# markomih/SplatFields

Measured on AMD Instinct MI355X. Metric: splats*px rasterized/sec (fwd+bwd), higher is better.
Workload: dtype f32

## Files before the change

include/splatraster.h:

```cpp
#ifndef SPLATRASTER_H
#define SPLATRASTER_H

#include <stddef.h>

#ifdef __cplusplus
extern "C" {
#endif

#define SR_VERSION 4
#define SR_TILE 16

typedef struct SrView {
    int image_height;
    int image_width;
    float tanfovx;
    float tanfovy;
    float scale_modifier;
    int sh_degree;
    int sh_coeffs;
    int prefiltered;
    int debug;
    const float* viewmatrix;
    const float* projmatrix;
    const float* campos;
// ... 21 lines not shown
typedef struct SrGrads {
    float* dL_dmeans3D;
    float* dL_dmeans2D;
    float* dL_dopacity;
    float* dL_dscales;
    float* dL_drotations;
    float* dL_dcov3D;
    float* dL_dshs;
    float* dL_dcolors;
    float* dL_dshs_rest;
} SrGrads;

int sr_version(void);
const char* sr_last_error(void);

size_t sr_geom_bytes(int n_splats, int height, int width);
size_t sr_binning_bytes(long long instances, int height, int width);
size_t sr_image_bytes(int height, int width);
size_t sr_backward_scratch_bytes(long long instances);

int sr_forward_prepare(const SrView* view, const SrSplats* splats, void* geom, int* radii,
                       long long* instances_out, void* hip_stream);

int sr_forward_render(const SrView* view, const SrSplats* splats, void* geom, void* binning,
                      long long instances, void* image, float* out_color, float* out_depth,
                      float* out_alpha, void* hip_stream);

#define SR_NEED_CAPACITY 2
int sr_forward(const SrView* view, const SrSplats* splats, void* geom, int* radii, void* binning,
               long long binning_capacity, void* image, float* out_color, float* out_depth, float* out_alpha,
               long long* instances_out, void* hip_stream);

int sr_forward_async(const SrView* view, const SrSplats* splats, void* geom, int* radii, void* binning,
                     long long binning_capacity, long long longest_list_hint, long long longest_list_expected, void* image,
                     float* out_color, float* out_depth, float* out_alpha, void** ticket_out, void* hip_stream);
int sr_ticket_wait(void* ticket, long long* instances_out, long long* longest_list_out);
long long sr_last_longest_list(void);
int sr_ticket_release(void* ticket);

#define SR_BWD_SLOT_SPEC_BELOW 6
int sr_backward(const SrView* view, const SrSplats* splats, const void* geom, void* binning,
                long long instances, long long instances_rendered, const void* image, const int* radii,
                const float* dL_dcolor, const float* dL_ddepth, const float* dL_dalpha, void* scratch,
                const SrGrads* grads, void* hip_stream);

int sr_backward_blend(const SrView* view, const SrSplats* splats, const void* geom, void* binning,
                      long long instances, long long instances_rendered, const void* image,
                      const float* dL_dcolor, const float* dL_ddepth, const float* dL_dalpha, void* scratch, void* hip_stream);
int sr_backward_splats(const SrView* view, const SrSplats* splats, const void* geom, void* binning,
                       long long instances, long long instances_rendered, const void* image, const int* radii, void* scratch,
                       const SrGrads* grads, int first_splat, int n_splats, void* hip_stream);

int sr_set_backward_kernel(int which);

int sr_mark_visible(int n_splats, const float* means3D, const float* viewmatrix,
                    const float* projmatrix, unsigned char* present, void* hip_stream);

int sr_densification_stats(int n_splats, const float* dL_dmeans2D, const int* radii, float* grad_accum, float* denom,
                           float* max_radii2D, void* hip_stream);

size_t sr_loss_workspace_bytes(int planes, int height, int width);
size_t sr_loss_maps_bytes(int planes, int height, int width);
int sr_photometric_forward(int batch, int channels, int height, int width, const float* image, const float* gt,
                           const float* alpha, const float* gt_mask, float lambda_dssim, float lambda_mask, void* workspace,
                           float* maps, float* loss, float* l1, float* ssim, float* mask_l1, void* hip_stream);
int sr_photometric_backward(int batch, int channels, int height, int width, const float* image, const float* gt,
                            const float* alpha, const float* gt_mask, const float* maps, float w_l1, float w_ssim, float w_mask,
                            const float* upstream, int upstream_per_item, float* dL_dimage, float* dL_dalpha, void* hip_stream);

#define SR_QUANT_NONE 0
#define SR_QUANT_PNG 1
#define SR_QUANT_TO8B 2
size_t sr_metrics_workspace_bytes(int batch, int height, int width);
int sr_image_metrics(int batch, int height, int width, const float* pred, const long long* pred_strides4, const float* gt,
                     const long long* gt_strides4, const float* mask, long long mask_item_stride, int quantize, void* workspace,
                     float* psnr, float* ssim, float* psnr_channels, unsigned char* frames, void* hip_stream);

int sr_sh_forward(int n_splats, int sh_coeffs, int sh_degree, const float* means3D, const float* shs, const float* campos,
                  float* colors, unsigned char* clamped, void* hip_stream);

int sr_sh_forward_views(int n_splats, int sh_coeffs, int sh_degree, int n_views, const float* means3D, const float* shs,
                        const float* campos, float* colors, float* keep, void* hip_stream);

int sr_sh_backward(int n_splats, int sh_coeffs, int sh_degree, int n_views, const float* means3D, const float* shs,
                   const float* campos, const float* dL_dcolors, float scale, float* dL_dshs, float* dL_dmeans3D,
                   int accumulate_means, void* hip_stream);

size_t sr_knn_workspace_bytes(int n_points);
int sr_knn3_mean_dist2(int n_points, const float* points, float* mean_dist2, void* workspace, void* hip_stream);

#define SR_KNN_MAX_K 8
size_t sr_knn_graph_workspace_bytes(int n_points, int k);
int sr_knn_graph(int n_points, int k, const float* points, int* nn_ix, unsigned* order, unsigned* rev_start, unsigned* rev_edges,
                 void* workspace, void* hip_stream);

#define SR_MORAN_MAX_TENSORS 8
size_t sr_moran_workspace_bytes(int n_items, int n_tensors);
size_t sr_moran_edges_bytes(int n_items, int k, int channels);
int sr_moran_forward(int n_items, int k, float eps, const float* points, const float* weight, const int* nn_ix,
                     const unsigned* order, int n_tensors, const float* const* features, const int* widths, void* workspace,
                     float* out, void* hip_stream);
int sr_moran_backward(int n_items, int k, float eps, const float* points, const float* weight, const int* nn_ix,
                      const unsigned* order, const unsigned* rev_start, const unsigned* rev_edges, int n_tensors,
                      const float* const* features, const int* widths, const float* out, const float* upstream, void* edges,
                      float* const* dL_dfeatures, float* dL_dpoints, float* dL_dweight, void* hip_stream);
int sr_moran_weights(int n_points, int k, float eps, const float* points, const int* nn_ix, float* weights, void* hip_stream);
// ... 200 lines not shown
```

splatfields_amd/_lib.py:

```python
from __future__ import annotations

import ctypes as C
from pathlib import Path

import os

import torch

LIB_PATH = Path(os.environ.get("SPLATRASTER_LIB") or (Path(__file__).resolve().parent / "libsplatraster.so"))

c_float_p = C.c_void_p


class SrView(C.Structure):
    _fields_ = [("image_height", C.c_int), ("image_width", C.c_int), ("tanfovx", C.c_float), ("tanfovy", C.c_float),
                ("scale_modifier", C.c_float), ("sh_degree", C.c_int), ("sh_coeffs", C.c_int), ("prefiltered", C.c_int),
                ("debug", C.c_int), ("viewmatrix", C.c_void_p), ("projmatrix", C.c_void_p), ("campos", C.c_void_p),
                ("bg", C.c_void_p)]


class SrSplats(C.Structure):
    _fields_ = [("count", C.c_int), ("means3D", C.c_void_p), ("opacities", C.c_void_p), ("scales", C.c_void_p),
                ("rotations", C.c_void_p), ("cov3D_precomp", C.c_void_p), ("shs", C.c_void_p),
                ("colors_precomp", C.c_void_p), ("raw_params", C.c_int), ("shs_rest", C.c_void_p)]
# ... 38 lines not shown

class SrPlaneJob(C.Structure):
    _fields_ = [(name, C.c_void_p) for name in (
        "x", "weight", "bias", "gamma", "beta", "stats", "residual", "out", "pre", "dy", "dx", "dweight", "dbias", "dgamma", "dbeta",
        "d_residual", "add", "dx_out")]


class SrHullView(C.Structure):
    _fields_ = [("m", C.c_double * 12), ("mask_offset", C.c_longlong), ("height", C.c_int), ("width", C.c_int),
                ("convention", C.c_int), ("outside", C.c_int)]


HULL_KRT, HULL_NDC, HULL_OUTSIDE_CARVE, HULL_OUTSIDE_KEEP, HULL_MAX_VIEWS = 0, 1, 0, 1, 1024
RESFIELD_MAX_JOBS, RESFIELD_MAX_RANK = 16, 64
PLANE_MAX_JOBS = 8
CONV_PROLOGUE, CONV_UPSAMPLE, CONV_RESIDUAL, CONV_SILU_OUT = 1, 2, 4, 8
MLP_MAX_GRAD_JOBS, MLP_MAX_GRAD_TASKS = 16, 128
MLP_MAX_PACK_JOBS = 32
MORAN_MAX_TENSORS, KNN_MAX_K = 8, 8
ADAM_MAX_TENSORS = 32
QUANT_NONE, QUANT_PNG, QUANT_TO8B = 0, 1, 2
MLP_MAX_OPS, MLP_NONE, MLP_LEAKY, MLP_MASK = 24, 0, 1, 2


SYMBOLS = {
    "sr_version": (C.c_int, []),
    "sr_last_error": (C.c_char_p, []),
    "sr_geom_bytes": (C.c_size_t, [C.c_int, C.c_int, C.c_int]),
    "sr_binning_bytes": (C.c_size_t, [C.c_longlong, C.c_int, C.c_int]),
    "sr_image_bytes": (C.c_size_t, [C.c_int, C.c_int]),
    "sr_backward_scratch_bytes": (C.c_size_t, [C.c_longlong]),
    "sr_forward_prepare": (C.c_int, [C.POINTER(SrView), C.POINTER(SrSplats), C.c_void_p, C.c_void_p,
                                     C.POINTER(C.c_longlong), C.c_void_p]),
    "sr_forward_render": (C.c_int, [C.POINTER(SrView), C.POINTER(SrSplats), C.c_void_p, C.c_void_p, C.c_longlong,
                                    C.c_void_p, C.c_void_p, C.c_void_p, C.c_void_p, C.c_void_p]),
    "sr_forward": (C.c_int, [C.POINTER(SrView), C.POINTER(SrSplats), C.c_void_p, C.c_void_p, C.c_void_p, C.c_longlong,
                             C.c_void_p, C.c_void_p, C.c_void_p, C.c_void_p, C.POINTER(C.c_longlong), C.c_void_p]),
    "sr_forward_async": (C.c_int, [C.POINTER(SrView), C.POINTER(SrSplats), C.c_void_p, C.c_void_p, C.c_void_p, C.c_longlong,
                                   C.c_longlong, C.c_longlong, C.c_void_p, C.c_void_p, C.c_void_p, C.c_void_p, C.POINTER(C.c_void_p),
                                   C.c_void_p]),
    "sr_ticket_wait": (C.c_int, [C.c_void_p, C.POINTER(C.c_longlong), C.POINTER(C.c_longlong)]),
    "sr_ticket_release": (C.c_int, [C.c_void_p]),
    "sr_last_longest_list": (C.c_longlong, []),
    "sr_debug_counters": (C.c_int, [C.POINTER(C.c_longlong), C.c_int]),
    "sr_backward": (C.c_int, [C.POINTER(SrView), C.POINTER(SrSplats), C.c_void_p, C.c_void_p, C.c_longlong, C.c_longlong, C.c_void_p,
                              C.c_void_p, C.c_void_p, C.c_void_p, C.c_void_p, C.c_void_p, C.POINTER(SrGrads),
                              C.c_void_p]),
    "sr_backward_blend": (C.c_int, [C.POINTER(SrView), C.POINTER(SrSplats), C.c_void_p, C.c_void_p, C.c_longlong, C.c_longlong, C.c_void_p,
                                    C.c_void_p, C.c_void_p, C.c_void_p, C.c_void_p, C.c_void_p]),
    "sr_backward_splats": (C.c_int, [C.POINTER(SrView), C.POINTER(SrSplats), C.c_void_p, C.c_void_p, C.c_longlong, C.c_longlong, C.c_void_p, C.c_void_p,
                                     C.c_void_p, C.POINTER(SrGrads), C.c_int, C.c_int, C.c_void_p]),
    "sr_debug_snapshot": (C.c_int, [C.POINTER(SrView), C.POINTER(SrSplats), C.c_void_p, C.c_void_p, C.c_void_p, C.c_int]),
    "sr_set_backward_kernel": (C.c_int, [C.c_int]),
    "sr_sh_forward": (C.c_int, [C.c_int, C.c_int, C.c_int, C.c_void_p, C.c_void_p, C.c_void_p, C.c_void_p, C.c_void_p, C.c_void_p]),
    "sr_sh_forward_views": (C.c_int, [C.c_int, C.c_int, C.c_int, C.c_int, C.c_void_p, C.c_void_p, C.c_void_p, C.c_void_p, C.c_void_p, C.c_void_p]),
    "sr_sh_backward": (C.c_int, [C.c_int, C.c_int, C.c_int, C.c_int, C.c_void_p, C.c_void_p, C.c_void_p, C.c_void_p, C.c_float,
                                 C.c_void_p, C.c_void_p, C.c_int, C.c_void_p]),
    "sr_knn_workspace_bytes": (C.c_size_t, [C.c_int]),
    "sr_knn3_mean_dist2": (C.c_int, [C.c_int, C.c_void_p, C.c_void_p, C.c_void_p, C.c_void_p]),
    "sr_knn_graph_workspace_bytes": (C.c_size_t, [C.c_int, C.c_int]),
    "sr_knn_graph": (C.c_int, [C.c_int, C.c_int, C.c_void_p, C.c_void_p, C.c_void_p, C.c_void_p, C.c_void_p, C.c_void_p, C.c_void_p]),
    "sr_moran_workspace_bytes": (C.c_size_t, [C.c_int, C.c_int]),
    "sr_moran_edges_bytes": (C.c_size_t, [C.c_int, C.c_int, C.c_int]),
    "sr_moran_forward": (C.c_int, [C.c_int, C.c_int, C.c_float, C.c_void_p, C.c_void_p, C.c_void_p, C.c_void_p, C.c_int,
                                   C.POINTER(C.c_void_p), C.POINTER(C.c_int), C.c_void_p, C.c_void_p, C.c_void_p]),
    "sr_moran_backward": (C.c_int, [C.c_int, C.c_int, C.c_float, C.c_void_p, C.c_void_p, C.c_void_p, C.c_void_p, C.c_void_p, C.c_void_p,
                                    C.c_int, C.POINTER(C.c_void_p), C.POINTER(C.c_int), C.c_void_p, C.c_void_p, C.c_void_p,
                                    C.POINTER(C.c_void_p), C.c_void_p, C.c_void_p, C.c_void_p]),
    "sr_moran_weights": (C.c_int, [C.c_int, C.c_int, C.c_float, C.c_void_p, C.c_void_p, C.c_void_p, C.c_void_p]),
    "sr_moran_weights_backward": (C.c_int, [C.c_int, C.c_int, C.c_float, C.c_void_p, C.c_void_p, C.c_void_p, C.c_void_p, C.c_void_p,
                                            C.c_void_p, C.c_void_p, C.c_void_p]),
    "sr_loss_workspace_bytes": (C.c_size_t, [C.c_int, C.c_int, C.c_int]),
    "sr_loss_maps_bytes": (C.c_size_t, [C.c_int, C.c_int, C.c_int]),
    "sr_photometric_forward": (C.c_int, [C.c_int, C.c_int, C.c_int, C.c_int, C.c_void_p, C.c_void_p, C.c_void_p, C.c_void_p, C.c_float,
                                         C.c_float, C.c_void_p, C.c_void_p, C.c_void_p, C.c_void_p, C.c_void_p, C.c_void_p, C.c_void_p]),
    "sr_photometric_backward": (C.c_int, [C.c_int, C.c_int, C.c_int, C.c_int, C.c_void_p, C.c_void_p, C.c_void_p, C.c_void_p, C.c_void_p,
                                          C.c_float, C.c_float, C.c_float, C.c_void_p, C.c_int, C.c_void_p, C.c_void_p, C.c_void_p]),
    "sr_metrics_workspace_bytes": (C.c_size_t, [C.c_int, C.c_int, C.c_int]),
    "sr_image_metrics": (C.c_int, [C.c_int, C.c_int, C.c_int, C.c_void_p, C.POINTER(C.c_longlong), C.c_void_p, C.POINTER(C.c_longlong),
                                   C.c_void_p, C.c_longlong, C.c_int, C.c_void_p, C.c_void_p, C.c_void_p, C.c_void_p, C.c_void_p,
                                   C.c_void_p]),
    "sr_adam_step": (C.c_int, [C.c_int, C.POINTER(SrAdamJob), C.c_void_p, C.c_longlong, C.c_void_p]),
    "sr_splat_reg_workspace_bytes": (C.c_size_t, [C.c_int]),
    "sr_splat_reg_forward": (C.c_int, [C.c_int, C.c_void_p, C.c_void_p, C.c_double, C.c_double, C.c_double, C.c_void_p, C.c_void_p, C.c_void_p]),
    "sr_splat_reg_backward": (C.c_int, [C.c_int, C.c_void_p, C.c_void_p, C.c_double, C.c_double, C.c_double, C.c_void_p, C.c_void_p, C.c_void_p,
                                        C.c_void_p, C.c_void_p]),
    "sr_depth_l1_workspace_bytes": (C.c_size_t, [C.c_int, C.c_int, C.c_int]),
    "sr_depth_l1_forward": (C.c_int, [C.c_int, C.c_int, C.c_int, C.c_void_p, C.c_void_p, C.c_void_p, C.c_void_p, C.c_void_p]),
    "sr_depth_l1_backward": (C.c_int, [C.c_int, C.c_int, C.c_int, C.c_void_p, C.c_void_p, C.c_void_p, C.c_int, C.c_void_p, C.c_void_p]),
    "sr_densify_workspace_bytes": (C.c_size_t, [C.c_int]),
    "sr_densify_plan": (C.c_int, [C.c_int, C.c_void_p, C.c_int, C.c_void_p, C.c_void_p, C.c_void_p, C.c_void_p, C.c_float, C.c_float,
                                  C.c_float, C.c_float, C.c_float, C.c_void_p, C.c_void_p, C.POINTER(C.c_longlong), C.c_void_p]),
    "sr_densify_gather": (C.c_int, [C.c_int, C.c_int, C.c_void_p, C.c_void_p, C.c_void_p, C.c_int, C.c_void_p, C.c_int, C.c_void_p,
                                    C.c_void_p, C.c_void_p]),
    "sr_hull_workspace_bytes": (C.c_size_t, [C.c_longlong]),
    "sr_hull_carve": (C.c_int, [C.c_int, C.POINTER(SrHullView), C.c_void_p, C.c_longlong, C.c_void_p, C.c_int, C.c_void_p, C.c_longlong,
                                C.c_int, C.c_void_p, C.c_void_p, C.c_void_p]),
    "sr_hull_gather": (C.c_int, [C.c_void_p, C.c_int, C.c_void_p, C.c_longlong, C.c_int, C.c_void_p, C.c_longlong, C.c_void_p, C.c_void_p,
                                 C.c_void_p]),
    "sr_mlp_pack": (C.c_int, [C.c_int, C.POINTER(SrMlpPackJob), C.c_void_p]),
    "sr_mlp_weight_grad_workspace": (C.c_size_t, [C.c_int, C.c_int, C.POINTER(SrMlpGradJob)]),
    "sr_mlp_weight_grad": (C.c_int, [C.c_int, C.c_int, C.POINTER(SrMlpGradJob), C.c_void_p, C.c_size_t, C.c_void_p]),
    "sr_mlp_chain": (C.c_int, [C.c_int, C.c_int, C.c_int, C.POINTER(SrMlpOp), C.c_float, C.c_void_p]),
    "sr_mlp_pack_bf16": (C.c_int, [C.c_int, C.POINTER(SrMlpPackJob), C.c_void_p]),
    "sr_mlp_chain_bf16": (C.c_int, [C.c_int, C.c_int, C.c_int, C.POINTER(SrMlpOp), C.c_float, C.c_void_p]),
    "sr_mlp_input_forward": (C.c_int, [C.c_int, C.c_int, C.c_int, C.c_int, C.c_int, C.c_void_p, C.c_void_p, C.c_void_p, C.c_void_p, C.c_void_p]),
# ... 95 lines not shown
```

splatfields_amd/csrc/api.hip:

```cpp
#include <cstdint>
#include <cstdio>
#include <cstdlib>
#include <cstring>
#include <atomic>
#include <chrono>
#include <thread>
#include <mutex>
#include <string>
#include <vector>
#include "kernels.h"

namespace {

thread_local std::string g_last_error;
thread_local long long g_last_longest = -1;

int fail(const std::string& msg) { g_last_error = msg; return 1; }

int check_hip(hipError_t e, const char* what) {
    if (e == hipSuccess) return 0;
    return fail(std::string(what) + ": " + hipGetErrorString(e));
}

template <typename... P>
// ... 405 lines not shown
    const sr::SplatsK& s = c.s;
    float* slots = static_cast<float*>(scratch);
    if (what & 1) {
        StageTimer t_(5, st);
        const int pinned = g_bwd_kernel.load(std::memory_order_relaxed);
        const bool wave_kernel = pinned == 1;
        if (wave_kernel) sr::launch_render_backward(c.v, c.g, c.b, c.im, dL_dcolor, dL_ddepth, dL_dalpha, slots, st);
        else sr::launch_render_backward_quads(c.v, c.g, c.b, c.im, dL_dcolor, dL_ddepth, dL_dalpha, slots, st);
    }
    if (what & 1) SR_TRY(after_launch(view, st, "render_backward"));
    if (what & 2) {
        sr::GradsK gr;
        gr.means3D = grads->dL_dmeans3D; gr.means2D = grads->dL_dmeans2D; gr.opacity = grads->dL_dopacity;
        gr.scales = s.cov3D ? nullptr : grads->dL_dscales; gr.rotations = s.cov3D ? nullptr : grads->dL_drotations;
        gr.cov3D = s.cov3D ? grads->dL_dcov3D : nullptr;
        gr.shs = s.shs ? grads->dL_dshs : nullptr;
        gr.shs_rest = (s.shs_rest && gr.shs) ? grads->dL_dshs_rest : nullptr;
        gr.colors = (s.colors || (s.shs && !grads->dL_dshs)) ? grads->dL_dcolors : nullptr;
        const bool small_fp = !(instances_rendered >= 0 && instances_rendered > (long long)SR_BWD_SLOT_SPEC_BELOW * (long long)s.N);
        { StageTimer t_(6, st); sr::launch_preprocess_backward(c.v, s, c.g, radii, slots, c.b.reached, gr, first, count, small_fp, st); }
        SR_TRY(after_launch(view, st, "preprocess_backward"));
    }
    return 0;
}
}

int sr_backward(const SrView* view, const SrSplats* splats, const void* geom, void* binning,
                long long instances, long long instances_rendered, const void* image, const int* radii,
                const float* dL_dcolor, const float* dL_ddepth, const float* dL_dalpha, void* scratch,
                const SrGrads* grads, void* hip_stream) {
    return backward_impl(3, view, splats, geom, binning, instances, instances_rendered, image, radii, dL_dcolor, dL_ddepth, dL_dalpha,
                         scratch, grads, 0, splats ? splats->count : 0, hip_stream);
}

int sr_backward_blend(const SrView* view, const SrSplats* splats, const void* geom, void* binning,
                      long long instances, long long instances_rendered, const void* image,
                      const float* dL_dcolor, const float* dL_ddepth, const float* dL_dalpha, void* scratch, void* hip_stream) {
    return backward_impl(1, view, splats, geom, binning, instances, instances_rendered, image, nullptr, dL_dcolor, dL_ddepth, dL_dalpha,
                         scratch, nullptr, 0, 0, hip_stream);
}

int sr_backward_splats(const SrView* view, const SrSplats* splats, const void* geom, void* binning,
                       long long instances, long long instances_rendered, const void* image, const int* radii, void* scratch,
                       const SrGrads* grads, int first_splat, int n_splats, void* hip_stream) {
    return backward_impl(2, view, splats, geom, binning, instances, instances_rendered, image, radii, nullptr, nullptr, nullptr, scratch,
                         grads, first_splat, n_splats, hip_stream);
}

int sr_set_backward_kernel(int which) {
    if (which < 0 || which > 2) return -1;
    return g_bwd_kernel.exchange(which, std::memory_order_relaxed);
}

int sr_mark_visible(int n, const float* means3D, const float* viewmatrix, const float*, unsigned char* present, void* hip_stream) {
    if (n < 0 || (n > 0 && (!means3D || !viewmatrix || !present))) return fail("bad arguments to sr_mark_visible");
    hipStream_t st = static_cast<hipStream_t>(hip_stream);
    sr::launch_mark_visible(n, means3D, viewmatrix, present, st);
    return check_hip(hipGetLastError(), "mark_visible");
}

int sr_densification_stats(int n, const float* dL_dmeans2D, const int* radii, float* grad_accum, float* denom, float* max_radii2D,
                           void* hip_stream) {
    if (n < 0) return fail("bad arguments to sr_densification_stats");
    if (n > 0 && (!dL_dmeans2D || !radii)) return fail("null pointer in sr_densification_stats");
    sr::launch_densification_stats(n, dL_dmeans2D, radii, grad_accum, denom, max_radii2D, static_cast<hipStream_t>(hip_stream));
    return check_hip(hipGetLastError(), "densification_stats");
}

int sr_sh_forward(int n, int sh_coeffs, int sh_degree, const float* means3D, const float* shs, const float* campos,
                  float* colors, unsigned char* clamped, void* hip_stream) {
    if (n < 0 || sh_degree < 0 || sh_degree > 3 || sh_coeffs < (sh_degree + 1) * (sh_degree + 1)) return fail("bad arguments to sr_sh_forward");
    if (n > 0 && (!means3D || !shs || !campos || !colors || !clamped)) return fail("null pointer in sr_sh_forward");
    sr::launch_sh_forward(n, sh_coeffs, sh_degree, means3D, shs, campos, colors, clamped, static_cast<hipStream_t>(hip_stream));
    return check_hip(hipGetLastError(), "sh_forward");
}

int sr_sh_forward_views(int n, int sh_coeffs, int sh_degree, int n_views, const float* means3D, const float* shs, const float* campos,
                        float* colors, float* keep, void* hip_stream) {
    if (n < 0 || n_views < 0 || sh_degree < 0 || sh_degree > 3 || sh_coeffs < (sh_degree + 1) * (sh_degree + 1)) return fail("bad arguments to sr_sh_forward_views");
    if (n > 0 && n_views > 0 && (!means3D || !shs || !campos || !colors)) return fail("null pointer in sr_sh_forward_views");
    sr::launch_sh_forward_views(n, sh_coeffs, sh_degree, n_views, means3D, shs, campos, colors, keep, static_cast<hipStream_t>(hip_stream));
    return check_hip(hipGetLastError(), "sh_forward_views");
}

int sr_sh_backward(int n, int sh_coeffs, int sh_degree, int n_views, const float* means3D, const float* shs, const float* campos,
                   const float* dL_dcolors, float scale, float* dL_dshs, float* dL_dmeans3D, int accumulate_means, void* hip_stream) {
    if (n < 0 || n_views < 0 || sh_degree < 0 || sh_degree > 3 || sh_coeffs < (sh_degree + 1) * (sh_degree + 1)) return fail("bad arguments to sr_sh_backward");
    if (n > 0 && n_views > 0 && (!means3D || !shs || !campos || !dL_dcolors)) return fail("null pointer in sr_sh_backward");
    sr::launch_sh_backward(n, sh_coeffs, sh_degree, n_views, means3D, shs, campos, dL_dcolors, scale, dL_dshs, dL_dmeans3D, accumulate_means,
                           static_cast<hipStream_t>(hip_stream));
    return check_hip(hipGetLastError(), "sh_backward");
}

size_t sr_knn_workspace_bytes(int n) { return sr::knn_workspace_bytes(n); }

int sr_knn3_mean_dist2(int n, const float* points, float* mean_dist2, void* workspace, void* hip_stream) {
    if (n < 0 || (n > 0 && (!points || !mean_dist2 || !workspace))) return fail("bad arguments to sr_knn3_mean_dist2");
    sr::launch_knn3(n, points, mean_dist2, workspace, static_cast<hipStream_t>(hip_stream));
    return check_hip(hipGetLastError(), "knn3");
}

size_t sr_knn_graph_workspace_bytes(int n, int k) { return sr::knn_graph_workspace_bytes(n, k); }

int sr_knn_graph(int n, int k, const float* points, int* nn_ix, unsigned* order, unsigned* rev_start, unsigned* rev_edges, void* workspace,
                 void* hip_stream) {
    if (n <= 0) return fail("bad arguments to sr_knn_graph: sizes must be positive");
// ... 579 lines not shown
```

splatfields_amd/csrc/binning.hip:

```cpp
#include <atomic>
#include "kernels.h"
#include "expand.h"

namespace sr {

static void allow_dynamic_lds(const void* kernel, int slot, int bytes) {
    static std::atomic<bool> done[8][64];
    int dev = 0;
    if (hipGetDevice(&dev) != hipSuccess) return;
    if (dev >= 0 && dev < 64 && done[slot][dev].load(std::memory_order_acquire)) return;
    if (hipFuncSetAttribute(kernel, hipFuncAttributeMaxDynamicSharedMemorySize, bytes) != hipSuccess) { (void)hipGetLastError(); return; }
    if (dev >= 0 && dev < 64) done[slot][dev].store(true, std::memory_order_release);
}

__global__ void __launch_bounds__(kBlock) k_count_tiles(const ViewK v, int N, const Geom g, const Chunking ch) {
    extern __shared__ __attribute__((aligned(16))) uint32_t s_hist[];
    __shared__ uint32_t s_off[kBlock + 1];
    __shared__ ushort4 s_rect[kBlock];
    __shared__ float4 s_r0[kBlock], s_r1[kBlock];
    __shared__ uint32_t s_scan[8];
    for (int t = 4 * threadIdx.x; t < ch.tiles_padded; t += 4 * kBlock) *reinterpret_cast<uint4*>(&s_hist[t]) = make_uint4(0u, 0u, 0u, 0u);
    __syncthreads();
    const int base_chunk = (int)blockIdx.x / ch.slices, slice = (int)blockIdx.x % ch.slices;
    const int sb0 = base_chunk * ch.sub_per_chunk, sb1 = min(sb0 + ch.sub_per_chunk, ch.n_sub);
    for (int sb = sb0; sb < sb1; ++sb) {
        const int idx = sb * kBlock + threadIdx.x;
        uint32_t touched = 0;
        ushort4 rect = make_ushort4(0, 0, 0, 0);
        float4 r0 = make_float4(0.f, 0.f, -1.f, 0.f), r1 = r0;
        if (idx < N) {
            touched = g.touched[idx]; rect = g.rect[idx];
            if (touched > kMaskTiles) { r0 = g.rec[4 * (size_t)idx]; r1 = g.rec[4 * (size_t)idx + 1]; }
        }
        const uint32_t mask = rect_mask16(rect);
        const ushort4 packed = rect;
        rect = rect_clean(rect);
        const bool direct = ch.slices == 1 && touched <= kDirectTiles;
        if (direct && touched > 0u) {
            uint32_t k = 0;
            for (uint32_t ty = rect.y; ty < rect.w; ++ty)
                for (uint32_t tx = rect.x; tx < rect.z; ++tx, ++k)
                    if ((mask >> k) & 1u) atomicAdd(&s_hist[ty * (uint32_t)v.gx + tx], 1u);
        }
        const uint32_t coop = direct ? 0u : touched;
        if (!__syncthreads_or(coop != 0u)) continue;
        uint32_t total;
        const uint32_t excl = block_exclusive_scan(coop, s_scan, total);
        s_off[threadIdx.x] = excl;
        s_rect[threadIdx.x] = packed;
        tile_test_prepare(r0, r1, s_r0[threadIdx.x], s_r1[threadIdx.x]);
        if (threadIdx.x == 0) s_off[kBlock] = total;
        __syncthreads();
        for_each_block_instance(s_off, s_rect, v.gx, [&](int e, uint32_t k, uint32_t tile, uint32_t, uint32_t tile_x, uint32_t tile_y, uint32_t w) {
// ... 469 lines not shown
        const uint32_t start = g.tile_start[tile];
        const uint32_t n = g.tile_start[tile + 1] - start;
        if (n <= (uint32_t)LO || n > (uint32_t)CAP) continue;
        sort_block_lds<CAP, THREADS>(b, start, n, run_key, [&](uint32_t rank, uint64_t key) { b.sorted_id[start + rank] = (uint32_t)key; });
    }
}

template <typename T>
__device__ __forceinline__ T ld_agent(const T* p) { return __hip_atomic_load(p, __ATOMIC_RELAXED, __HIP_MEMORY_SCOPE_AGENT); }

template <int CAP, int THREADS>
__global__ void __launch_bounds__(THREADS) k_sort_tiles_long(const Geom g, const Binning b, int n_tiles) {
    extern __shared__ __attribute__((aligned(16))) unsigned char s_dyn[];
    uint64_t* run_key = reinterpret_cast<uint64_t*>(s_dyn);
    if (g.total[0] > b.capacity) return;
    const uint32_t limit = min((uint32_t)n_tiles, g.total[6]);
    for (uint32_t slot = blockIdx.x; slot < limit; slot += gridDim.x) {
        const uint32_t tile = g.tile_order[slot];
        const uint32_t start = g.tile_start[tile];
        const uint32_t n = g.tile_start[tile + 1] - start;
        if (n <= (uint32_t)CAP) continue;
        uint64_t* k0 = b.keys + start;
        uint64_t* k1 = b.keys_tmp + start;
        for (uint32_t c0 = 0; c0 < n; c0 += CAP) {
            const uint32_t m = min((uint32_t)CAP, n - c0);
            sort_block_lds<CAP, THREADS>(b, start + c0, m, run_key, [&](uint32_t rank, uint64_t key) { k0[c0 + rank] = key; });
        }
        for (uint32_t width = CAP; width < n; width <<= 1) {
            __threadfence();
            __syncthreads();
            for (uint32_t i = threadIdx.x; i < n; i += THREADS) {
                const uint32_t pair_base = (i / (2 * width)) * (2 * width);
                const uint32_t mid = min(pair_base + width, n), end = min(pair_base + 2 * width, n);
                const bool left = i < mid;
                const uint64_t key = ld_agent(k0 + i);
                uint32_t lo = left ? mid : pair_base, hi = left ? end : mid;
                while (lo < hi) {
                    const uint32_t mm = (lo + hi) >> 1;
                    if (ld_agent(k0 + mm) < key) lo = mm + 1; else hi = mm;
                }
                const uint32_t rank = lo - (left ? mid : pair_base);
                const uint32_t pos = pair_base + (i - (left ? pair_base : mid)) + rank;
                k1[pos] = key;
            }
            uint64_t* tk = k0; k0 = k1; k1 = tk;
        }
        __threadfence();
        __syncthreads();
        for (uint32_t i = threadIdx.x; i < n; i += THREADS) b.sorted_id[start + i] = (uint32_t)ld_agent(k0 + i);
        __syncthreads();
    }
}

void launch_sort_tiles(const ViewK& v, const Geom& g, const Binning& b, long long max_len, long long expected_len, hipStream_t st) {
    const int tiles = v.gx * v.gy;
    if (tiles <= 0) return;
    auto lds = [](int cap, int) { return (size_t)cap * 16; };
    hipLaunchKernelGGL(k_sort_tiles_regs, dim3(tiles), dim3(256), 0, st, g, b);
    if (max_len >= 0 && max_len <= 2048) return;
    allow_dynamic_lds(reinterpret_cast<const void*>(&k_sort_tiles_merge<2048, 4096, 1024>), 2, (int)lds(4096, 1024));
    allow_dynamic_lds(reinterpret_cast<const void*>(&k_sort_tiles_merge<4096, 8192, 1024>), 3, (int)lds(8192, 1024));
    allow_dynamic_lds(reinterpret_cast<const void*>(&k_sort_tiles_long<8192, 1024>), 4, (int)lds(8192, 1024));
    const int long_grid = tiles < 512 ? tiles : 512;
    auto grid_for = [&](long long lo) { return (expected_len >= 0 && expected_len <= lo) ? (long_grid < 8 ? long_grid : 8) : long_grid; };
    hipLaunchKernelGGL((k_sort_tiles_merge<2048, 4096, 1024>), dim3(grid_for(2048)), dim3(1024), lds(4096, 1024), st, g, b, tiles);
    if (max_len >= 0 && max_len <= 4096) return;
    hipLaunchKernelGGL((k_sort_tiles_merge<4096, 8192, 1024>), dim3(grid_for(4096)), dim3(1024), lds(8192, 1024), st, g, b, tiles);
    if (max_len >= 0 && max_len <= 8192) return;
    hipLaunchKernelGGL((k_sort_tiles_long<8192, 1024>), dim3(grid_for(8192)), dim3(1024), lds(8192, 1024), st, g, b, tiles);
}

}
```

splatfields_amd/csrc/kernels.h:

```cpp
#pragma once
#include "common.h"

namespace sr {

struct SplatsK {
    int N;
    const float* means3D; const float* opacities; const float* scales; const float* rotations;
    const float* cov3D; const float* shs; const float* colors;
    int raw;
    const float* shs_rest;
};

struct GradsK {
    float* means3D; float* means2D; float* opacity; float* scales; float* rotations; float* cov3D;
    float* shs; float* colors; float* shs_rest;
};

void launch_preprocess(const ViewK& v, const SplatsK& s, const Geom& g, int* radii, hipStream_t st);
void launch_mark_visible(int N, const float* means3D, const float* viewmatrix, unsigned char* present, hipStream_t st);
void launch_densification_stats(int N, const float* dL_dmeans2D, const int* radii, float* grad_accum, float* denom, float* max_radii2D,
                                hipStream_t st);
void launch_preprocess_backward(const ViewK& v, const SplatsK& s, const Geom& g, const int* radii,
                                const float* slots, const uint8_t* reached, const GradsK& gr, int first, int count, bool small_footprint,
                                hipStream_t st);
inline bool use_count_matrix(const ViewK& v) { return v.gx * v.gy <= kMaxMatrixTiles; }
void launch_count_tiles(const ViewK& v, int N, const Geom& g, hipStream_t st);
void launch_scan_small(const ViewK& v, int N, const Geom& g, uint32_t* host_out, uint32_t host_seq, hipStream_t st);
void launch_emit(const ViewK& v, int N, const Geom& g, const Binning& b, hipStream_t st);
void launch_sort_tiles(const ViewK& v, const Geom& g, const Binning& b, long long max_len, long long expected_len, hipStream_t st);
void launch_render_forward(const ViewK& v, const Geom& g, const Binning& b, const Image& im,
                           float* out_color, float* out_depth, float* out_alpha, hipStream_t st);
void launch_render_backward(const ViewK& v, const Geom& g, const Binning& b, const Image& im,
                            const float* dL_dcolor, const float* dL_ddepth, const float* dL_dalpha,
                            float* slots, hipStream_t st);
void launch_render_backward_quads(const ViewK& v, const Geom& g, const Binning& b, const Image& im,
                                 const float* dL_dcolor, const float* dL_ddepth, const float* dL_dalpha,
                                 float* slots, hipStream_t st);

int backward_stats(unsigned long long* out8, int reset);

struct DensifyArgs { float grad_threshold, min_opacity, extent, percent_dense, max_screen_size; };
size_t densify_workspace_bytes(int n);
void launch_densify_plan(int n, const float* log_scales, int scale_cols, const float* opacity_logit, const float* grad_accum,
                         const float* denom, const float* max_radii2D, const DensifyArgs& a, void* workspace, int32_t* dest,
                         uint32_t** totals_out, hipStream_t st);
void launch_densify_gather(int n, int row, const float* src, float* dst, const int32_t* dest, int mode, const float* log_scales,
                           int scale_cols, const float* rotations, const float* unit, hipStream_t st);

size_t hull_workspace_bytes(long long n);
hipError_t launch_hull_carve(int n_views, const SrHullView* host_views, const uint8_t* masks, const double* grid, int G, const void* points,
                             long long n, int point_is_double, void* workspace, int* count_out, hipStream_t st);
void launch_hull_gather(const double* grid, int G, const void* points, long long n, int point_is_double, const void* workspace,
                        long long capacity, int* indices_out, float* points_out, hipStream_t st);

size_t mlp_weight_grad_workspace(int n_points, int n_jobs, const SrMlpGradJob* jobs);
int launch_mlp_weight_grad(int n_points, int n_jobs, const SrMlpGradJob* jobs, void* workspace, size_t workspace_bytes, hipStream_t st);
int launch_mlp_pack(int n_jobs, const SrMlpPackJob* jobs, bool bf16, hipStream_t st);
int launch_mlp_chain(int n_points, int hidden_tiles, int n_ops, const SrMlpOp* ops, float slope, bool bf16, hipStream_t st);

int launch_mlp_input_forward(int N, int L, int F, int TL, int row, const float* xyz, const float* feat, const float* time, float* x0, hipStream_t st);
int launch_mlp_top_gradient(int N, int out, int row, const float* y, const float* dy, float slope, float* G, hipStream_t st);
int launch_mlp_input_backward(int N, int L, int F, int row, const float* xyz, const float* g, float* d_xyz, float* d_feat, hipStream_t st);
int launch_resfield_compose(int n_jobs, const SrResFieldJob* jobs, const long long* frame, hipStream_t st);
size_t resfield_backward_workspace(int n_jobs, const SrResFieldJob* jobs);
int launch_resfield_backward(int n_jobs, const SrResFieldJob* jobs, const long long* frame, void* workspace, size_t workspace_bytes, hipStream_t st);

int launch_triplane_forward(int N, int C, int H, int W, const float* planes_chw, float* planes_hwc, const float* pts, float* out, hipStream_t st);
int launch_triplane_backward(int N, int C, int H, int W, const float* planes_hwc, const float* pts, const float* g, float* d_planes_chw,
                             float* d_pts, void* workspace, hipStream_t st);
size_t triplane_backward_workspace(int N, int C, int H, int W);

size_t knn_workspace_bytes(int n);
void launch_knn3(int n, const float* pts, float* out, void* workspace, hipStream_t st);
constexpr int kKnnMinK = 2, kKnnMaxK = 8;
size_t knn_graph_workspace_bytes(int n, int k);
void launch_knn_graph(int n, int k, const float* pts, int* nn_ix, uint32_t* order, uint32_t* rev_start, uint32_t* rev_edges, void* workspace,
                      hipStream_t st);

constexpr int kMoranMaxTensors = SR_MORAN_MAX_TENSORS;
struct MoranTensors {
    int count, channels, edge_channels;
    const float* x[kMoranMaxTensors]; float* dx[kMoranMaxTensors];
// ... 66 lines not shown
```

splatfields_amd/rasterizer.py:

```python
from __future__ import annotations

import contextlib
import ctypes as C
import math
import os
import threading
import weakref
from typing import NamedTuple, Optional

import torch
from torch import nn

from . import _lib


class GaussianRasterizationSettings(NamedTuple):
    image_height: int
    image_width: int
    tanfovx: float
    tanfovy: float
    bg: torch.Tensor
    scale_modifier: float
    viewmatrix: torch.Tensor
    projmatrix: torch.Tensor
# ... 25 lines not shown
    return _DEPTH_GRADIENT

_ASYNC = {"1": True, "true": True, "True": True, "on": True, "0": False, "false": False, "False": False, "off": False}.get(
    os.environ.get("SPLATRASTER_ASYNC", ""), None)
_HEADROOM = 1.25


class RasterizerOverflow(RuntimeError):
    """An asynchronously launched forward (sr_forward_async) met more tile-splat instances, or a longer tile list, than the
    last render of that view had promised: it has no result (its outputs are NaN).  The estimates have been corrected; render
    again."""


def set_async_forward(enabled) -> "Optional[bool]":
    global _ASYNC
    prev, _ASYNC = _ASYNC, (None if enabled is None else bool(enabled))
    return prev


class async_forward:

    def __init__(self, enabled: bool = True):
        self.enabled = bool(enabled)

    def __enter__(self):
        self.prev = getattr(_TLS, "async_scope", None)
        _TLS.async_scope = self.enabled
        return self

    def __exit__(self, *exc):
        _TLS.async_scope = self.prev
        return False


def async_forward_enabled() -> bool:
    if _ASYNC is not None:
        return _ASYNC
    return bool(getattr(_TLS, "async_scope", None))


def host_sync_counters(reset: bool = False) -> dict:
    out = (C.c_longlong * 4)()
    _lib.check(_lib.load().sr_debug_counters(out, 1 if reset else 0))
    return {"forward_host_waits": int(out[0]), "async_forwards": int(out[1]), "tickets_waited_for": int(out[2]),
            "tickets_created": int(out[3])}


_BWD_KERNELS = {None: 0, "auto": 0, "wave": 1, "quads": 2}


def set_backward_kernel(which) -> str:
    prev = _lib.load().sr_set_backward_kernel(_BWD_KERNELS[which])
    return {0: "auto", 1: "wave", 2: "quads"}[prev]


def _round_capacity(instances: int) -> int:
    c = max(int(instances * _HEADROOM) + 1024, 1 << 16)
    step = 1 << (c.bit_length() - 4)
    return (c + step - 1) // step * step


def _covered_by_hint(hint: int) -> int:
    return 2048 if hint <= 2048 else 4096 if hint <= 4096 else 8192 if hint <= 8192 else 1 << 62


class _Promise(NamedTuple):
    key: tuple
    capacity: int
    hint: Optional[int] = None
    expected: int = -1
    covered: int = 0


class _Estimates:

    CAPACITY_ROWS = 4096
    SEEN_ROWS = 64

    def __init__(self):
        self.capacity = {}
        self.per_splat = {}
        self.lock = threading.Lock()

    def plan(self, device_index: int, n: int, H: int, W: int, view, may_async: bool) -> _Promise:
        key = (device_index, n, H, W)
        with self.lock:
            ratio = self.per_splat.get((device_index, H, W))
            capacity = self.capacity.get(key) or (max(4 * n, 1 << 16) if ratio is None else _round_capacity(int(ratio * n)))
            before = view.seen.get(n) if may_async else None
        if before is None or _round_capacity(before[0]) > capacity:
            return _Promise(key, capacity)
        hint = int(before[1] * _HEADROOM) + 1
        return _Promise(key, capacity, hint, int(before[1]), _covered_by_hint(hint))

    def record(self, promise: _Promise, view, instances: int, longest: int) -> None:
        global LAST_INSTANCES
        dev, n, H, W = key = promise.key
        rkey = (dev, H, W)
        with self.lock:
            self.capacity[key] = max(self.capacity.get(key, 0), _round_capacity(instances))
            if len(self.capacity) > self.CAPACITY_ROWS:
                self.capacity.clear()
            self.per_splat[rkey] = max(self.per_splat.get(rkey, 0.0), instances / max(n, 1))
            if longest >= 0:
                if len(view.seen) > self.SEEN_ROWS:
                    view.seen.clear()
# ... 478 lines not shown
```

Before: 1310000 billion.

## Add LDS radix sort for long per-tile lists replacing merge pass up to 4096

```diff
diff --git a/include/splatraster.h b/include/splatraster.h
--- a/include/splatraster.h
+++ b/include/splatraster.h
@@ -97,6 +97,8 @@
                        const SrGrads* grads, int first_splat, int n_splats, void* hip_stream);
 
 int sr_set_backward_kernel(int which);
+
+int sr_set_sort_kernel(int which);
 
 int sr_mark_visible(int n_splats, const float* means3D, const float* viewmatrix,
                     const float* projmatrix, unsigned char* present, void* hip_stream);
diff --git a/splatfields_amd/_lib.py b/splatfields_amd/_lib.py
--- a/splatfields_amd/_lib.py
+++ b/splatfields_amd/_lib.py
@@ -114,6 +114,7 @@
                                      C.c_void_p, C.POINTER(SrGrads), C.c_int, C.c_int, C.c_void_p]),
     "sr_debug_snapshot": (C.c_int, [C.POINTER(SrView), C.POINTER(SrSplats), C.c_void_p, C.c_void_p, C.c_void_p, C.c_int]),
     "sr_set_backward_kernel": (C.c_int, [C.c_int]),
+    "sr_set_sort_kernel": (C.c_int, [C.c_int]),
     "sr_sh_forward": (C.c_int, [C.c_int, C.c_int, C.c_int, C.c_void_p, C.c_void_p, C.c_void_p, C.c_void_p, C.c_void_p, C.c_void_p]),
     "sr_sh_forward_views": (C.c_int, [C.c_int, C.c_int, C.c_int, C.c_int, C.c_void_p, C.c_void_p, C.c_void_p, C.c_void_p, C.c_void_p, C.c_void_p]),
     "sr_sh_backward": (C.c_int, [C.c_int, C.c_int, C.c_int, C.c_int, C.c_void_p, C.c_void_p, C.c_void_p, C.c_void_p, C.c_float,
diff --git a/splatfields_amd/csrc/api.hip b/splatfields_amd/csrc/api.hip
--- a/splatfields_amd/csrc/api.hip
+++ b/splatfields_amd/csrc/api.hip
@@ -481,6 +481,11 @@
     return g_bwd_kernel.exchange(which, std::memory_order_relaxed);
 }
 
+int sr_set_sort_kernel(int which) {
+    if (which < 0 || which > 2) return -1;
+    return sr::set_sort_kernel(which);
+}
+
 int sr_mark_visible(int n, const float* means3D, const float* viewmatrix, const float*, unsigned char* present, void* hip_stream) {
     if (n < 0 || (n > 0 && (!means3D || !viewmatrix || !present))) return fail("bad arguments to sr_mark_visible");
     hipStream_t st = static_cast<hipStream_t>(hip_stream);
diff --git a/splatfields_amd/csrc/binning.hip b/splatfields_amd/csrc/binning.hip
--- a/splatfields_amd/csrc/binning.hip
+++ b/splatfields_amd/csrc/binning.hip
@@ -1,4 +1,7 @@
 #include <atomic>
+#include <cstdio>
+#include <cstdlib>
+#include <string>
 #include "kernels.h"
 #include "expand.h"
 
@@ -574,18 +577,279 @@
     }
 }
 
+constexpr int kRadixCap = 4096;
+constexpr uint32_t kRadixTieRun = 8;
+#ifndef SR_SORT_RADIX_FROM
+#define SR_SORT_RADIX_FROM 2049
+#endif
+
+__device__ __forceinline__ uint32_t radix_p0(uint32_t C) {
+    uint32_t p0 = (threadIdx.x >> 6) * C + (threadIdx.x & 63u);
+    asm volatile("" : "+v"(p0));
+    return p0;
+}
+
+struct RadixLds {
+    uint64_t* keys;
+    uint16_t* hist;
+    uint32_t* misc;
+    uint32_t parity;
+};
+
+template <int E>
+__device__ __forceinline__ void radix_pass(uint64_t (&k)[E], RadixLds& s, bool hi_word, uint32_t shift, uint32_t bits, uint32_t n, uint32_t C) {
+    const uint32_t lane = threadIdx.x & 63u, w = threadIdx.x >> 6;
+    uint32_t p0;
+    const uint32_t dmask = (1u << bits) - 1u;
+    uint16_t* hist = s.hist + s.parity * 1024u;
+    uint16_t* hist_next = s.hist + (s.parity ^ 1u) * 1024u;
+    uint16_t* row = hist + w * 256u;
+    auto digit = [&](uint64_t key) { return ((hi_word ? (uint32_t)(key >> 32) : (uint32_t)key) >> shift) & dmask; };
+    uint32_t off[E];
+    p0 = radix_p0(C);
+#pragma unroll
+    for (int e = 0; e < E; ++e) {
+        if ((uint32_t)e * 64u < C) {
+            const uint32_t nd = ~digit(k[e]);
+            const uint64_t in_range = __builtin_amdgcn_ballot_w64(p0 + (uint32_t)e * 64u < n);
+            uint32_t peers_lo = (uint32_t)in_range, peers_hi = (uint32_t)(in_range >> 32);
+            for (uint32_t i = 0; i < bits; ++i) {
+                const uint32_t m = (uint32_t)__builtin_amdgcn_sbfe((int)nd, i, 1u);
+                const uint64_t bal = __builtin_amdgcn_ballot_w64(m == 0u);
+                peers_lo &= (uint32_t)bal ^ m; peers_hi &= (uint32_t)(bal >> 32) ^ m;
+            }
+            const uint32_t below = __builtin_amdgcn_mbcnt_hi(peers_hi, __builtin_amdgcn_mbcnt_lo(peers_lo, 0u));
+            off[e] = below | ((uint32_t)(__popc(peers_lo) + __popc(peers_hi)) << 16);
+        }
+    }
+    p0 = radix_p0(C);
+#pragma unroll
+    for (int e = 0; e < E; ++e) {
+        if ((uint32_t)e * 64u < C) {
+            const bool valid = p0 + (uint32_t)e * 64u < n;
+            const uint32_t d = digit(k[e]);
+            const uint32_t before = row[d], below = off[e] & 0xffffu;
+            __builtin_amdgcn_wave_barrier();
+            if (valid && below == 0u) row[d] = (uint16_t)(before + (off[e] >> 16));
+            __builtin_amdgcn_wave_barrier();
+            off[e] = before + below;
+        }
+    }
+    __syncthreads();
+    const uint32_t t = threadIdx.x;
+    const uint32_t c0 = hist[t], c1 = hist[256u + t], c2 = hist[512u + t], c3 = hist[768u + t];
+    const uint32_t tot = c0 + c1 + c2 + c3;
+    uint32_t inc = tot;
+#pragma unroll
+    for (int d = 1; d < 64; d <<= 1) {
+        const uint32_t up = __shfl_up(inc, d, 64);
+        if (lane >= (uint32_t)d) inc += up;
+    }
+    if (lane == 63u) s.misc[w] = inc;
+    hist_next[t] = 0; hist_next[256u + t] = 0; hist_next[512u + t] = 0; hist_next[768u + t] = 0;
+    __syncthreads();
+    uint32_t base = inc - tot;
+    for (uint32_t ww = 0; ww < w; ++ww) base += s.misc[ww];
+    hist[t] = (uint16_t)base; hist[256u + t] = (uint16_t)(base + c0);
+    hist[512u + t] = (uint16_t)(base + c0 + c1); hist[768u + t] = (uint16_t)(base + c0 + c1 + c2);
+    __syncthreads();
+    p0 = radix_p0(C);
+#pragma unroll
+    for (int e = 0; e < E; ++e) {
+        const uint32_t p = p0 + (uint32_t)e * 64u;
+        if ((uint32_t)e * 64u < C && p < n) {
+            const uint32_t pos = row[digit(k[e])] + off[e];
+            if (pos < n) s.keys[pos] = k[e];
+        }
+    }
+    __syncthreads();
+    p0 = radix_p0(C);
+#pragma unroll
+    for (int e = 0; e < E; ++e) {
+        const uint32_t p = p0 + (uint32_t)e * 64u;
+        if ((uint32_t)e * 64u < C) k[e] = p < n ? s.keys[p] : 0ull;
+    }
+    s.parity ^= 1u;
+}
+
+template <int E>
+__device__ __forceinline__ void radix_or_and(const uint64_t (&k)[E], RadixLds& s, bool hi_word, uint32_t n, uint32_t C, uint32_t& vor, uint32_t& vand) {
+    const uint32_t lane = threadIdx.x & 63u, w = threadIdx.x >> 6;
+    uint32_t p0;
+    vor = 0u; vand = ~0u;
+    p0 = radix_p0(C);
+#pragma unroll
+    for (int e = 0; e < E; ++e) {
+        const uint32_t p = p0 + (uint32_t)e * 64u;
+        if ((uint32_t)e * 64u < C && p < n) {
+            const uint32_t word = hi_word ? (uint32_t)(k[e] >> 32) : (uint32_t)k[e];
+            vor |= word; vand &= word;
+        }
+    }
+    vor |= lane_xor<1>(vor); vand &= lane_xor<1>(vand);
+    vor |= lane_xor<2>(vor); vand &= lane_xor<2>(vand);
+    vor |= lane_xor<4>(vor); vand &= lane_xor<4>(vand);
+    vor |= lane_xor<8>(vor); vand &= lane_xor<8>(vand);
+    vor |= lane_xor<16>(vor); vand &= lane_xor<16>(vand);
+    vor |= lane_xor<32>(vor); vand &= lane_xor<32>(vand);
+    if (lane == 0u) { s.misc[4u + w] = vor; s.misc[8u + w] = vand; }
+    __syncthreads();
+    vor = __builtin_amdgcn_readfirstlane(s.misc[4] | s.misc[5] | s.misc[6] | s.misc[7]);
+    vand = __builtin_amdgcn_readfirstlane(s.misc[8] & s.misc[9] & s.misc[10] & s.misc[11]);
+}
+
+template <int E>
+__device__ __forceinline__ void radix_word(uint64_t (&k)[E], RadixLds& s, bool hi_word, uint32_t vor, uint32_t vand, uint32_t n, uint32_t C) {
+    const uint32_t diff = __builtin_amdgcn_readfirstlane(vor ^ vand);
+    if (diff == 0u) return;
+    const uint32_t lo = (uint32_t)__builtin_ctz(diff), hi = 32u - (uint32_t)__builtin_clz(diff);
+    const uint32_t passes = (hi - lo + 7u) / 8u, bits = (hi - lo + passes - 1u) / passes;
+    for (uint32_t shift = lo; shift < hi; shift += bits) radix_pass<E>(k, s, hi_word, shift, min(bits, hi - shift), n, C);
+}
+
+template <int E>
+__device__ __forceinline__ void load_radix(const Binning& b, uint32_t start, uint32_t n, uint32_t C, uint64_t (&k)[E]) {
+    const uint32_t p0 = radix_p0(C);
+#pragma unroll
+    for (int e = 0; e < E; ++e) {
+        const uint32_t p = p0 + (uint32_t)e * 64u;
+        k[e] = ((uint32_t)e * 64u < C && p < n) ? b.ent[start + p] : 0ull;
+    }
+}
+
+template <int E>
+__device__ __forceinline__ void sort_tile_radix(const Binning& b, uint32_t start, uint32_t n, RadixLds s) {
+    uint32_t p0;
+    const uint32_t C = ((n + 3u) / 4u + 63u) & ~63u;
+    uint64_t k[E];
+    {
+        uint32_t* h32 = reinterpret_cast<uint32_t*>(s.hist);
+#pragma unroll
+        for (int i = 0; i < 4; ++i) h32[threadIdx.x + 256u * i] = 0u;
+        if (threadIdx.x == 0u) s.misc[12] = 0u;
+    }
+    s.parity = 0u;
+    uint32_t vor[2] = {0u, 0u}, vand[2] = {0u, 0u};
+    for (uint32_t attempt = 0u;; ++attempt) {
+        load_radix<E>(b, start, n, C, k);
+        const uint32_t first_word = 1u - attempt;
+        radix_or_and<E>(k, s, first_word == 1u, n, C, vor[first_word], vand[first_word]);
+        for (uint32_t word = first_word; word < 2u; ++word) radix_word<E>(k, s, word == 1u, vor[word], vand[word], n, C);
+        if (attempt == 1u) {
+            p0 = radix_p0(C);
+#pragma unroll
+            for (int e = 0; e < E; ++e) k[e] = ((uint64_t)(p0 + (uint32_t)e * 64u) << 32) | (uint32_t)k[e];
+            break;
+        }
+        if (vor[1] == vand[1]) {
+            p0 = radix_p0(C);
+#pragma unroll
+            for (int e = 0; e < E; ++e) {
+                const uint32_t p = p0 + (uint32_t)e * 64u;
+                if ((uint32_t)e * 64u < C && p < n) s.keys[p] = k[e];
+            }
+            __syncthreads();
+        }
+        bool long_run = false;
+        p0 = radix_p0(C);
+#pragma unroll
+        for (int e = 0; e < E; ++e) {
+            const uint32_t p = p0 + (uint32_t)e * 64u;
+            if ((uint32_t)e * 64u < C && p < n) {
+                const uint32_t d = (uint32_t)(k[e] >> 32), id = (uint32_t)k[e];
+                uint32_t before = 0u, after = 0u, less = 0u;
+                for (uint32_t j = 1u; j <= kRadixTieRun && j <= p; ++j) {
+                    const uint64_t o = s.keys[p - j];
+                    if ((uint32_t)(o >> 32) != d) break;
+                    ++before; less += (uint32_t)o < id ? 1u : 0u;
+                }
+                for (uint32_t j = 1u; j <= kRadixTieRun && p + j < n; ++j) {
+                    const uint64_t o = s.keys[p + j];
+                    if ((uint32_t)(o >> 32) != d) break;
+                    ++after; less += (uint32_t)o < id ? 1u : 0u;
+                }
+                long_run |= before == kRadixTieRun || after == kRadixTieRun;
+                k[e] = ((uint64_t)(p - before + less) << 32) | id;
+            }
+        }
+        if (long_run) s.misc[12] = 1u;
+        __syncthreads();
+        if (__builtin_amdgcn_readfirstlane(s.misc[12]) == 0u) break;
+    }
+    p0 = radix_p0(C);
+#pragma unroll
+    for (int e = 0; e < E; ++e) {
+        const uint32_t p = p0 + (uint32_t)e * 64u;
+        const uint32_t rank = (uint32_t)(k[e] >> 32);
+        if ((uint32_t)e * 64u < C && p < n && rank < n) b.sorted_id[start + rank] = (uint32_t)k[e];
+    }
+}
+
+template <int CAP>
+__global__ void __launch_bounds__(256) __attribute__((amdgpu_waves_per_eu(CAP > 2048 ? 4 : 6))) k_sort_tiles_radix(const Geom g, const Binning b, uint32_t radix_from) {
+    constexpr uint32_t cap = (uint32_t)CAP;
+    extern __shared__ __attribute__((aligned(16))) unsigned char s_dyn[];
+    uint64_t* skey = reinterpret_cast<uint64_t*>(s_dyn);
+    const uint32_t total_instances = g.total[0];
+    const uint32_t tile = g.tile_order[blockIdx.x];
+    asm volatile("" :: "s"(tile));
+    if (total_instances > b.capacity) return;
+    const uint32_t start = g.tile_start[tile];
+    const uint32_t n = g.tile_start[tile + 1] - start;
+    if (n == 0u || n > cap) return;
+    if (n < radix_from) {
+        if (n <= 256u) sort_tile_regs<256, 1>(b, start, n, skey);
+        else if (n <= 512u) sort_tile_regs<512, 2>(b, start, n, skey);
+        else if (n <= 1024u) sort_tile_regs<1024, 4>(b, start, n, skey);
+        else sort_block_lds<2048, 256>(b, start, n, skey, [&](uint32_t rank, uint64_t key) { b.sorted_id[start + rank] = (uint32_t)key; });
+        return;
+    }
+    RadixLds s;
+    s.keys = skey;
+    s.hist = reinterpret_cast<uint16_t*>(skey + cap);
+    s.misc = reinterpret_cast<uint32_t*>(s.hist + 2048);
+    if (CAP <= 2048 || n <= 2048u) sort_tile_radix<8>(b, start, n, s);
+    else sort_tile_radix<16>(b, start, n, s);
+}
+
+static std::atomic<int> g_sort_kernel{[] {
+    const char* sel = getenv("SPLATRASTER_SORT");
+    if (!sel || !*sel) return 0;
+    if (std::string(sel) == "bitonic") return 1;
+    if (std::string(sel) == "radix") return 2;
+    fprintf(stderr, "splatraster: SPLATRASTER_SORT=%s is neither \"bitonic\" nor \"radix\": the product choice is used\n", sel);
+    return 0;
+}()};
+int set_sort_kernel(int which) { return g_sort_kernel.exchange(which, std::memory_order_relaxed); }
+
 void launch_sort_tiles(const ViewK& v, const Geom& g, const Binning& b, long long max_len, long long expected_len, hipStream_t st) {
     const int tiles = v.gx * v.gy;
     if (tiles <= 0) return;
     auto lds = [](int cap, int) { return (size_t)cap * 16; };
-    hipLaunchKernelGGL(k_sort_tiles_regs, dim3(tiles), dim3(256), 0, st, g, b);
-    if (max_len >= 0 && max_len <= 2048) return;
+    const int pinned = g_sort_kernel.load(std::memory_order_relaxed);
+    constexpr uint32_t kProductFrom = (uint32_t)(SR_SORT_RADIX_FROM);
+    static_assert(kProductFrom <= 2049u, "the register network of k_sort_tiles_radix ends at 2048 entries");
+    const bool longer = !(max_len >= 0 && max_len <= 2048);
+    uint32_t cap = 0u;
+    if (pinned == 2) cap = longer ? (uint32_t)kRadixCap : 2048u;
+    else if (pinned == 0 && kProductFrom != 0u) cap = longer ? (uint32_t)kRadixCap : (kProductFrom <= 2048u ? 2048u : 0u);
+    if (cap != 0u) {
+        const uint32_t radix_from = pinned == 2 ? 1u : kProductFrom;
+        const size_t bytes = (size_t)cap * 8 + 2 * 4 * 256 * sizeof(uint16_t) + 16 * sizeof(uint32_t);
+        if (cap == 2048u) hipLaunchKernelGGL(k_sort_tiles_radix<2048>, dim3(tiles), dim3(256), bytes, st, g, b, radix_from);
+        else hipLaunchKernelGGL(k_sort_tiles_radix<kRadixCap>, dim3(tiles), dim3(256), bytes, st, g, b, radix_from);
+    } else {
+        hipLaunchKernelGGL(k_sort_tiles_regs, dim3(tiles), dim3(256), 0, st, g, b);
+    }
+    if (!longer) return;
+    if (max_len >= 0 && max_len <= (long long)cap) return;
     allow_dynamic_lds(reinterpret_cast<const void*>(&k_sort_tiles_merge<2048, 4096, 1024>), 2, (int)lds(4096, 1024));
     allow_dynamic_lds(reinterpret_cast<const void*>(&k_sort_tiles_merge<4096, 8192, 1024>), 3, (int)lds(8192, 1024));
     allow_dynamic_lds(reinterpret_cast<const void*>(&k_sort_tiles_long<8192, 1024>), 4, (int)lds(8192, 1024));
     const int long_grid = tiles < 512 ? tiles : 512;
     auto grid_for = [&](long long lo) { return (expected_len >= 0 && expected_len <= lo) ? (long_grid < 8 ? long_grid : 8) : long_grid; };
-    hipLaunchKernelGGL((k_sort_tiles_merge<2048, 4096, 1024>), dim3(grid_for(2048)), dim3(1024), lds(4096, 1024), st, g, b, tiles);
+    if (cap != (uint32_t)kRadixCap)
+        hipLaunchKernelGGL((k_sort_tiles_merge<2048, 4096, 1024>), dim3(grid_for(2048)), dim3(1024), lds(4096, 1024), st, g, b, tiles);
     if (max_len >= 0 && max_len <= 4096) return;
     hipLaunchKernelGGL((k_sort_tiles_merge<4096, 8192, 1024>), dim3(grid_for(4096)), dim3(1024), lds(8192, 1024), st, g, b, tiles);
     if (max_len >= 0 && max_len <= 8192) return;
diff --git a/splatfields_amd/csrc/kernels.h b/splatfields_amd/csrc/kernels.h
--- a/splatfields_amd/csrc/kernels.h
+++ b/splatfields_amd/csrc/kernels.h
@@ -28,6 +28,7 @@
 void launch_scan_small(const ViewK& v, int N, const Geom& g, uint32_t* host_out, uint32_t host_seq, hipStream_t st);
 void launch_emit(const ViewK& v, int N, const Geom& g, const Binning& b, hipStream_t st);
 void launch_sort_tiles(const ViewK& v, const Geom& g, const Binning& b, long long max_len, long long expected_len, hipStream_t st);
+int set_sort_kernel(int which);
 void launch_render_forward(const ViewK& v, const Geom& g, const Binning& b, const Image& im,
                            float* out_color, float* out_depth, float* out_alpha, hipStream_t st);
 void launch_render_backward(const ViewK& v, const Geom& g, const Binning& b, const Image& im,
diff --git a/splatfields_amd/rasterizer.py b/splatfields_amd/rasterizer.py
--- a/splatfields_amd/rasterizer.py
+++ b/splatfields_amd/rasterizer.py
@@ -101,6 +101,14 @@
 def set_backward_kernel(which) -> str:
     prev = _lib.load().sr_set_backward_kernel(_BWD_KERNELS[which])
     return {0: "auto", 1: "wave", 2: "quads"}[prev]
+
+
+_SORT_KERNELS = {None: 0, "auto": 0, "bitonic": 1, "radix": 2}
+
+
+def set_sort_kernel(which) -> str:
+    prev = _lib.load().sr_set_sort_kernel(_SORT_KERNELS[which])
+    return {0: "auto", 1: "bitonic", 2: "radix"}[prev]
 
 
 def _round_capacity(instances: int) -> int:
```

Result: no change. 1321000 billion (median of 6 runs) (+0.8%).
